# teshnizi/GraphEnvs

Measured on AMD Instinct MI355X. Metric: env-steps/sec (whole node), ShortestPath-v0 n=64 m=192 batch=65536, 1/2/4/8 GPU, higher is better.
Workload: dtype u64; 1 GPU; ShortestPath-v0 n_nodes=64 n_edges=192 weighted, 65536 env slots per GPU, random valid actions on device, same-step autoreset (seed-exact G(n,m)+features on device); envs_per_gpu=65536, prefetch_period=0, episodes_finished_per_gpu=6165512, settle_steps=128, parallelism=batch shard x1, no collective

## Files before the change

graphenvs_amd/csrc/ge_features.h:

```cpp
#pragma once
#include "ge_params.h"
#include "ge_platform.h"
#include "ge_reset.h"

struct GeFctx {
  uint64_t *abits; int *rowptr; uint16_t *scw;
  uint64_t *quads; uint32_t *rq; int zq;
  uint8_t *c8;
  double *sigma, *delta, *coeff, *bcw;
  double *bcw0; int wave_f64;
  double *bc, *clos;
  double *prx, *prn, *sinv, *diff, *diff2, *clus;
  uint8_t *mark;
  uint16_t *ord, *lvl;
};

GE_DEV GeFctx ge_carve_f(const GeParams &P, int tid) {
  unsigned char *s = ge_dyn_smem();
  const GeLdsF &L = P.ldsf;
  const int n = P.n, an = ((n * 8 + 15) & ~15) / 8;
  GeFctx c;
  c.rowptr = (int *)(s + L.rowptr); c.quads = (uint64_t *)(s + L.colw); c.c8 = (uint8_t *)(s + L.colw); c.rq = (uint32_t *)(s + L.rq); c.zq = L.zq;
  c.bc = (double *)(s + L.bc); c.clos = (double *)(s + L.clos);
  unsigned char *w = s + L.wave0 + (tid >> 6) * L.wave_stride;
  const int bcw_at = P.W <= GE_BCW_REG_W ? n : 3 * n + 1;
  c.sigma = (double *)(w + L.w_sigma); c.delta = c.sigma + n; c.coeff = c.sigma + 2 * n; c.bcw = c.sigma + bcw_at;
  c.mark = (uint8_t *)(w + L.w_mark); c.ord = (uint16_t *)(w + L.w_ord); c.lvl = (uint16_t *)(w + L.w_lvl);
  c.bcw0 = (double *)(s + L.wave0 + L.w_sigma) + bcw_at; c.wave_f64 = L.wave_stride / 8;
  c.abits = (uint64_t *)(s + L.abits); c.scw = (uint16_t *)(s + L.scw);
  c.prx = (double *)(s + L.prx); c.prn = c.prx + an; c.sinv = c.prx + 2 * an; c.diff = c.prx + 3 * an; c.diff2 = c.prx + 4 * an; c.clus = (double *)(s + L.clus);
  return c;
}

#ifndef GE_PR_CH
#define GE_PR_CH 4
#endif
#ifndef GE_FABL
#define GE_FABL 0
#endif
#if defined(GE_STAMPS) && !defined(GE_EMU)
#define GE_FSTAMP_DECL unsigned long long fs_acc[8] = {0, 0, 0, 0, 0, 0, 0, 0}, fs_t = clock64(), fs_src = 0, fs_lev = 0; int fs_k = 7
#define GE_FSTAMP(k) do { const unsigned long long now_ = clock64(); fs_acc[fs_k] += now_ - fs_t; fs_t = now_; fs_k = (k); if ((k) == 6) fs_src++; if ((k) == 1) fs_lev++; } while (0)
#define GE_FSTAMP_OUT do { if (env == 0 && part == 0 && tid == 0) { for (int k_ = 0; k_ < 8; k_++) ge_stamp_buf[16 + k_] = fs_acc[k_]; ge_stamp_buf[24] = fs_src; ge_stamp_buf[25] = fs_lev; } } while (0)
#else
#define GE_FSTAMP_DECL do { } while (0)
#define GE_FSTAMP(k) do { } while (0)
#define GE_FSTAMP_OUT do { } while (0)
#endif
GE_HOSTDEV int ge_feat_workgroups(int feat_parts) { return feat_parts > 1 ? feat_parts + 1 : 1; }
#ifndef GE_BW_TWO_ABOVE
#define GE_BW_TWO_ABOVE 256
#endif
#ifndef GE_BW_U
#define GE_BW_U 1
#endif
template <bool BWD, int U>
GE_DEV void ge_brandes_walk_u(const GeFctx &c, int k0, int k1, int lane, bool store) {
  for (int kb = k0; kb < k1; kb += U * GE_WAVE) {
    bool on[U]; int v[U]; uint32_t q0[U], nq[U]; double sv[U], acc[U]; uint64_t q[U];
#pragma unroll
    for (int u = 0; u < U; u++) { const int k = kb + u * GE_WAVE + lane; on[u] = k < k1; v[u] = (int)c.ord[on[u] ? k : k0]; }
#pragma unroll
    for (int u = 0; u < U; u++) { const uint32_t r = c.rq[v[u]]; q0[u] = r & 0xffffu; nq[u] = on[u] ? (r >> 16) : 0u; sv[u] = BWD ? c.sigma[v[u]] : 1.0; acc[u] = 0.0; }
#pragma unroll
    for (int u = 0; u < U; u++) q[u] = c.quads[nq[u] ? q0[u] : (uint32_t)c.zq];
    for (uint32_t i = 0; ge_ballot(i < nq[0] || (U > 1 && i < nq[U - 1])) != 0ull;) {
      i++;
      uint64_t qn[U];
#pragma unroll
      for (int u = 0; u < U; u++) qn[u] = c.quads[i < nq[u] ? q0[u] + i : (uint32_t)c.zq];
#pragma unroll
      for (int u = 0; u < U; u++) {
        const uint32_t lo = (uint32_t)q[u], hi = (uint32_t)(q[u] >> 32);
        const int w0 = (int)(lo & 0xffffu), w1 = (int)(lo >> 16), w2 = (int)(hi & 0xffffu), w3 = (int)(hi >> 16);
        const double f0 = c.coeff[w0], f1 = c.coeff[w1], f2 = c.coeff[w2], f3 = c.coeff[w3];
        if (!BWD) { c.mark[w0] = 1; c.mark[w1] = 1; c.mark[w2] = 1; c.mark[w3] = 1; }
        if (BWD) { acc[u] += sv[u] * f0; acc[u] += sv[u] * f1; acc[u] += sv[u] * f2; acc[u] += sv[u] * f3; }
        else { acc[u] += f0; acc[u] += f1; acc[u] += f2; acc[u] += f3; }
        q[u] = qn[u];
      }
    }
#pragma unroll
    for (int u = 0; u < U; u++) if (on[u] && store) (BWD ? c.delta : c.sigma)[v[u]] = acc[u];
  }
}
template <bool BWD>
GE_DEV void ge_brandes_walk(const GeFctx &c, int k0, int k1, int lane, bool store, bool two) {
  if (GE_BW_U > 1 && two && k1 - k0 > GE_WAVE) ge_brandes_walk_u<BWD, GE_BW_U>(c, k0, k1, lane, store); else ge_brandes_walk_u<BWD, 1>(c, k0, k1, lane, store);
}

GE_DEV void ge_features_generic_env(const GeParams &P, int env, int part, int nparts) {
  const int tid = ge_tid_fresh(), nthreads = ge_bdim();
  const int lane = tid & (GE_WAVE - 1), wv = tid >> 6, nwaves = P.ldsf.waves;
  const bool search_wave = wv < nwaves;
  const int n = P.n, W = P.W, E = P.E, F = P.F, t = P.env_type;
  const ge_buffers &G = P.buf;
  const int64_t nbase = (int64_t)env * n, ebase = (int64_t)env * E;
  GeFctx c = ge_carve_f(P, tid);
  const bool node_part = nparts > 1 && part == nparts;
  const bool node_role = node_part || nparts == 1, brandes_role = !node_part;
  if (node_role) { const uint64_t *arows = G.adj_bits + nbase * W; for (int i = tid; i < n * W; i += nthreads) c.abits[i] = arows[i]; }
  const bool closed = P.complete && P.ng == n;
  const bool trivial = closed || node_part;
  uint8_t *c8 = c.c8;
  const int32_t *grow = G.row_ptr + (int64_t)env * (n + 1);
  const uint16_t *gcolw = G.colw + ebase;
  for (int v = tid; v <= n; v += nthreads) c.rowptr[v] = grow[v];
  if (closed) { for (int idx = tid; idx < E; idx += nthreads) c8[idx] = G.scode[ebase + idx]; }
  else if (brandes_role) {
    uint16_t *q16 = (uint16_t *)c.quads;
    for (int v = tid; v < n; v += nthreads) {
      const int r0 = grow[v], r1 = grow[v + 1], q0 = (r0 + 3 * v) >> 2, nq = (r1 - r0 + 3) >> 2;
      c.rq[v] = (uint32_t)q0 | ((uint32_t)nq << 16);
      for (int i = 0; i < nq; i++) {
        uint32_t e[4];
#pragma unroll
        for (int j = 0; j < 4; j++) { const int k = r0 + 4 * i + j; const uint32_t x = gcolw[k < r1 ? k : r0]; e[j] = k < r1 ? (x >> 4) : (uint32_t)n; }
        c.quads[q0 + i] = (uint64_t)(e[0] | (e[1] << 16)) | ((uint64_t)(e[2] | (e[3] << 16)) << 32);
      }
    }
    if (tid < 4) q16[4 * c.zq + tid] = (uint16_t)n;
  }
  ge_sync();
  if (node_role && !closed) for (int v = tid; v < n; v += nthreads)
    for (int k = c.rowptr[v]; k < c.rowptr[v + 1]; k++) {
      const uint16_t e = gcolw[k];
      c.scw[c.rowptr[v] + ge_rank_below(c.abits + v * W, e >> 4)] = e;
    }
  const bool bcw_reg = W <= GE_BCW_REG_W;
  double bcr[GE_BCW_REG_W];
#pragma unroll
  for (int j = 0; j < GE_BCW_REG_W; j++) bcr[j] = 0.0;
  if (brandes_role && !bcw_reg && search_wave) for (int v = lane; v < n; v += GE_WAVE) c.bcw[v] = 0.0;
  ge_sync();
  if (trivial && !node_part) for (int v = tid; v < n; v += nthreads) c.clos[v] = (((double)n - 1.0) / (double)(n - 1)) * (((double)n - 1.0) / (double)(n - 1));
  const bool two = n > GE_BW_TWO_ABOVE;
  GE_FSTAMP_DECL;
  for (int s = part * nwaves + wv; s < n && !trivial && search_wave; s += nwaves * nparts) {
    GE_FSTAMP(6);
    for (int v = lane; v < n; v += GE_WAVE) { c.sigma[v] = (v == s) ? 1.0 : 0.0; c.delta[v] = 0.0; c.coeff[v] = (v == s) ? 1.0 : 0.0; c.mark[v] = 0; }
    const uint32_t rs = c.rq[s];
    const int deg_s = c.rowptr[s + 1] - c.rowptr[s];
    { const uint16_t *row = (const uint16_t *)(c.quads + (rs & 0xffffu)); for (int i = lane; i < deg_s; i += GE_WAVE) c.ord[1 + i] = row[i]; }
    if (lane == 0) { c.coeff[n] = 0.0; c.mark[n] = 0; c.ord[0] = (uint16_t)s; c.lvl[0] = 0; c.lvl[1] = 1; c.lvl[2] = (uint16_t)(1 + deg_s); }
    ge_wave_sync();
    int d = deg_s ? 1 : 0, reach = 1 + deg_s, lp = 0, lo = deg_s ? 1 : 0, hi = 1 + deg_s; int64_t tot = deg_s;
    const uint32_t *sig_hi = (const uint32_t *)c.sigma + 1;
    for (;;) {
      GE_FSTAMP(1);
      if (!(GE_FABL & 1) && d > 0) ge_brandes_walk<false>(c, lo, hi, lane, true, two);
      ge_wave_sync();
      GE_FSTAMP(0);
      int found = 0;
      for (int w0 = 0; w0 < n; w0 += 4 * GE_WAVE) {
        uint32_t m[4], sh[4];
#pragma unroll
        for (int j = 0; j < 4; j++) { const int w = w0 + GE_WAVE * j + lane; const bool in = w < n; m[j] = c.mark[in ? w : n]; sh[j] = sig_hi[2 * (in ? w : 0)]; }
#pragma unroll
        for (int j = 0; j < 4; j++) if (w0 + GE_WAVE * j < n) {
          const int w = w0 + GE_WAVE * j + lane; const bool in = w < n;
          const bool isnew = in && m[j] != 0u && sh[j] == 0u;
          const uint64_t b = ge_ballot(isnew);
          if (isnew) c.ord[hi + found + ge_mbcnt(b)] = (uint16_t)w;
          if (in) c.mark[w] = 0;
          found += ge_popc64(b);
        }
      }
      if (!found) break;
      for (int k = lp + lane; k < lo; k += GE_WAVE) c.coeff[c.ord[k]] = 0.0;
      for (int k = lo + lane; k < hi; k += GE_WAVE) { const int v = c.ord[k]; c.coeff[v] = c.sigma[v]; }
      d++; lp = lo; lo = hi; hi += found; reach += found; tot += (int64_t)d * found;
      if (lane == 0) c.lvl[d + 1] = (uint16_t)hi;
      ge_wave_sync();
    }
    for (int k = lp + lane; k < lo; k += GE_WAVE) c.coeff[c.ord[k]] = 0.0;
    ge_wave_sync();
    for (int lev = d; lev >= 2; lev--) {
      GE_FSTAMP(3);
      const int l0 = c.lvl[lev], l1 = c.lvl[lev + 1], l2 = lev < d ? (int)c.lvl[lev + 2] : l1, p0 = c.lvl[lev - 1];
      for (int k = l1 + lane; k < l2; k += GE_WAVE) c.coeff[c.ord[k]] = 0.0;
      for (int k = l0 + lane; k < l1 && !(GE_FABL & 2); k += GE_WAVE) { const int v = c.ord[k]; c.coeff[v] = (1.0 + c.delta[v]) / c.sigma[v]; if (!bcw_reg) c.bcw[v] += c.delta[v]; }
      ge_wave_sync();
      GE_FSTAMP(4);
      if (!(GE_FABL & 4)) ge_brandes_walk<true>(c, p0, l0, lane, true, two);
      ge_wave_sync();
    }
    GE_FSTAMP(5);
    if (!bcw_reg) { const int l1 = c.lvl[2]; for (int k = 1 + lane; k < l1; k += GE_WAVE) { const int v = c.ord[k]; c.bcw[v] += c.delta[v]; } }
    if (bcw_reg) {
#pragma unroll
      for (int j = 0; j < GE_BCW_REG_W; j++) { const int v = lane + GE_WAVE * j; if (j < W) bcr[j] += (v < n && v != s) ? c.delta[v] : 0.0; }
    }
    if (lane == 0) {
      double cc = 0.0;
      if (tot > 0 && n > 1) { cc = ((double)reach - 1.0) / (double)tot; double sc = ((double)reach - 1.0) / (double)(n - 1); cc *= sc; }
      c.clos[s] = cc;
    }
    ge_wave_sync();
  }
  GE_FSTAMP(7);
  GE_FSTAMP_OUT;
  if (bcw_reg && brandes_role && search_wave) {
#pragma unroll
    for (int j = 0; j < GE_BCW_REG_W; j++) { const int v = lane + GE_WAVE * j; if (j < W && v < n) c.bcw[v] = bcr[j]; }
  }
  ge_sync();
  if (brandes_role) for (int v = tid; v < n; v += nthreads) { double acc = 0.0; for (int w = 0; w < nwaves; w++) acc += c.bcw0[w * c.wave_f64 + v]; c.bc[v] = acc; }
  ge_sync();
  if (nparts > 1) {
    if (!node_part) {
      for (int v = tid; v < n; v += nthreads) G.feat_scratch[((int64_t)env * nparts + part) * n + v] = c.bc[v];
      for (int v = tid; v < n; v += nthreads) if ((v % (nwaves * nparts)) / nwaves == part) G.x[(nbase + v) * F + P.nflag + 2] = (float)c.clos[v];
      ge_sync();
      return;
    }
  }
  if (n > 2 && nparts == 1) { double scale = 1.0 / (double)((int64_t)(n - 1) * (int64_t)(n - 2)); for (int v = tid; v < n; v += nthreads) c.bc[v] *= scale; }
  double *clus = c.clus;
  for (int i = tid; i < n; i += nthreads) {
    int64_t common = 0, dg = c.rowptr[i + 1] - c.rowptr[i];
    for (int k = c.rowptr[i]; k < c.rowptr[i + 1]; k++) {
      int j;
      if (closed) { const int q = k - c.rowptr[i]; j = q < i ? q : q + 1; } else j = c.scw[k] >> 4;
      for (int w = 0; w < W; w++) common += ge_popc64(c.abits[i * W + w] & c.abits[j * W + w]);
    }
    int64_t t8 = 8 * common, dt = 2 * dg, db = dg;
    clus[i] = (t8 == 0) ? 0.0 : (double)t8 / (double)((dt * (dt - 1) - 2 * db) * 2);
  }
  const bool prw = (t == GE_TSP);
  const double pinit = 1.0 / (double)n;
  int ndang = 0;
  for (int k0 = 0; k0 < n; k0 += GE_WAVE) {
    int i = k0 + lane;
    ndang += ge_popc64(ge_ballot(i < n && c.rowptr[i + 1] == c.rowptr[i]));
  }
  double *wl = (double *)(ge_dyn_smem() + P.ldsf.wl);
  if (tid < 16) wl[tid] = ge_wlut(tid);
  ge_sync();
  for (int i = tid; i < n; i += nthreads) {
    double S = 0.0;
    for (int k = c.rowptr[i]; k < c.rowptr[i + 1]; k++) S += (prw ? (P.spatial ? G.sw64[ebase + k] : wl[closed ? (int)c8[k] : (int)(c.scw[k] & 15)]) : 1.0) * 1.0;
    c.sinv[i] = (S != 0.0) ? 1.0 / S : 0.0;
    c.prx[i] = pinit;
  }
  ge_sync();
  const double alpha = 0.85, oma = 1 - alpha, tol = 1.0e-6;
  double *xc = c.prx, *xw = c.prn, *dc = c.diff, *dw = c.diff2;
  bool conv = false;
  for (int it = 0; it < ((GE_FABL & 8) ? 1 : 100) && !conv; it++) {
    double dsum = 0.0;
    if (ndang) { bool first = true; for (int i = 0; i < n; i++) if (c.rowptr[i + 1] == c.rowptr[i]) { dsum = first ? xc[i] : dsum + xc[i]; first = false; } }
    for (int i = tid; i < n; i += nthreads) {
      double acc = 0.0;
      const int r0 = c.rowptr[i], r1 = c.rowptr[i + 1];
      for (int k0 = r0; k0 < r1; k0 += GE_PR_CH) {
        int jn[GE_PR_CH], cd[GE_PR_CH]; double sv[GE_PR_CH], xv[GE_PR_CH], wv[GE_PR_CH];
#pragma unroll
        for (int q = 0; q < GE_PR_CH; q++) {
          const int kk = k0 + q < r1 ? k0 + q : r0;
          if (closed) { const int qq = kk - r0; jn[q] = qq < i ? qq : qq + 1; cd[q] = (int)c8[kk]; }
          else { const uint32_t e = (uint32_t)c.scw[kk]; jn[q] = (int)(e >> 4); cd[q] = (int)(e & 15u); }
        }
#pragma unroll
        for (int q = 0; q < GE_PR_CH; q++) {
          sv[q] = c.sinv[jn[q]]; xv[q] = xc[jn[q]];
          wv[q] = prw ? (P.spatial ? G.sw64[ebase + (k0 + q < r1 ? k0 + q : r0)] : wl[cd[q]]) : 1.0;
        }
#pragma unroll
        for (int q = 0; q < GE_PR_CH; q++) if (k0 + q < r1) acc += (sv[q] * wv[q]) * xv[q];
      }
      double xn = alpha * (acc + dsum * pinit) + oma * pinit;
      xw[i] = xn;
      dc[i] = __builtin_fabs(xn - xc[i]);
    }
    ge_sync();
    const double err = ge_pw<5>(dc, n, lane);
    { double *t_ = xc; xc = xw; xw = t_; t_ = dc; dc = dw; dw = t_; }
    if (err < (double)n * tol) conv = true;
  }

  for (int v = tid; v < n; v += nthreads) {
    float *xr = G.x + (nbase + v) * F + P.nflag;
    xr[0] = (float)(2.0 * (double)(c.rowptr[v + 1] - c.rowptr[v]));
    if (nparts == 1) { xr[1] = (float)c.bc[v]; xr[2] = (float)c.clos[v]; }
    xr[3] = (float)xc[v]; xr[4] = (float)clus[v];
  }
  ge_sync();
}

#ifndef GE_F64_LV
#define GE_F64_LV 12
#endif
#ifndef GE_F64_INV
#define GE_F64_INV 128
#endif
#ifndef GE_F64_ABL
#define GE_F64_ABL 0
#endif
#ifndef GE_F64_U
#define GE_F64_U 2
#endif
#ifndef GE_F64_L2POP
#define GE_F64_L2POP 1
#endif
#define GE_F64_THREADS 256
#define GE_F64_WAVES 4
#define GE_F64_SB 8
#define GE_F64_LST 16
#define GE_F64_ITEMS 16
static_assert(GE_F64_LV + 1 <= GE_F64_LST, "level starts");
static_assert(GE_F64_INV <= 256, "path counts are kept as bytes");
#define GE_F64_SS 65
#define GE_F64_SG 68
#define GE_F64_A_S 0
#define GE_F64_A_SIG (GE_F64_A_S + GE_F64_SB * GE_F64_SS * 8)
#define GE_F64_A_LVL (GE_F64_A_SIG + GE_F64_SB * GE_F64_SG)
#define GE_F64_A_ORD (GE_F64_A_LVL + GE_F64_LV * GE_F64_SB * 8)
#define GE_F64_A_LST (GE_F64_A_ORD + GE_F64_SB * 64)
#define GE_F64_A_BYTES (GE_F64_A_LST + GE_F64_SB * GE_F64_LST)
#define GE_F64_W_INV 512
#define GE_F64_W_CLOS (GE_F64_W_INV + GE_F64_INV * 8)
#define GE_F64_W_AREA (GE_F64_W_CLOS + 512)
#define GE_F64_W_BYTES (GE_F64_W_AREA + GE_F64_WAVES * GE_F64_A_BYTES)

GE_HOSTDEV int ge_f64_node_wave_bytes(int E, int tsp) { return 512 + 4 * 512 + (tsp ? ((E + 15) & ~15) : 0); }
GE_HOSTDEV int ge_f64_pre_off(int E, int tsp, int nblk) {
  int o = GE_F64_W_BYTES;
  const int nd = GE_F64_WAVES * ge_f64_node_wave_bytes(E, tsp), pf = (nblk + 2) * 4;
  if (nd > o) o = nd;
  if (pf > o) o = pf;
  return (o + 15) & ~15;
}
GE_HOSTDEV int ge_f64_bytes(int E, int tsp, int nblk) { return ge_f64_pre_off(E, tsp, nblk) + GE_F64_ITEMS * 4 * 4 + 16; }

template <int BASE>
GE_DEV void ge_f64_next_bits(uint32_t &b, int (&idx)[GE_F64_U]) {
#pragma unroll
  for (int j = 0; j < GE_F64_U; j++) {
#ifdef GE_EMU
    idx[j] = b ? BASE + __builtin_ctz(b) : 64;
#else
    uint32_t z;
    asm("v_ffbl_b32 %0, %1" : "=v"(z) : "v"(b));
    idx[j] = (int)((z < (uint32_t)(64 - BASE) ? z : (uint32_t)(64 - BASE)) + (uint32_t)BASE);
#endif
    b &= b - 1u;
  }
}
GE_DEV uint32_t ge_f64_sum_counts(const uint8_t *row, uint64_t p) {
  uint32_t acc = 0u;
  for (uint32_t b = (uint32_t)p; b;) {
    int ix[GE_F64_U]; uint32_t r[GE_F64_U];
    ge_f64_next_bits<0>(b, ix);
#pragma unroll
    for (int j = 0; j < GE_F64_U; j++) r[j] = row[ix[j]];
#pragma unroll
    for (int j = 0; j < GE_F64_U; j++) acc += r[j];
  }
  for (uint32_t b = (uint32_t)(p >> 32); b;) {
    int ix[GE_F64_U]; uint32_t r[GE_F64_U];
    ge_f64_next_bits<32>(b, ix);
#pragma unroll
    for (int j = 0; j < GE_F64_U; j++) r[j] = row[ix[j]];
#pragma unroll
    for (int j = 0; j < GE_F64_U; j++) acc += r[j];
  }
  return acc;
}
#ifndef GE_F64_COEFF
#define GE_F64_COEFF 0
#endif
template <int BASE>
GE_DEV double ge_f64_sum_coeff_half(const uint8_t *sigrow, const double *Srow, const double *inv, uint32_t b, double acc) {
#if GE_F64_COEFF
  while (b) {
    int ix[GE_F64_U]; double sw[GE_F64_U];
    ge_f64_next_bits<BASE>(b, ix);
#pragma unroll
    for (int j = 0; j < GE_F64_U; j++) sw[j] = Srow[ix[j]];
#pragma unroll
    for (int j = 0; j < GE_F64_U; j++) acc += sw[j];
  }
  return acc;
#endif
  while (b) {
    int ix[GE_F64_U]; uint32_t sg[GE_F64_U]; double sw[GE_F64_U], iv[GE_F64_U];
    ge_f64_next_bits<BASE>(b, ix);
#pragma unroll
    for (int j = 0; j < GE_F64_U; j++) { sg[j] = sigrow[ix[j]]; sw[j] = Srow[ix[j]]; }
#pragma unroll
    for (int j = 0; j < GE_F64_U; j++) iv[j] = inv[sg[j]];
#pragma unroll
    for (int j = 0; j < GE_F64_U; j++) acc += iv[j] + sw[j];
  }
  return acc;
}

GE_DEV void ge_f64_walk_env(const GeParams &P, int env, int *ovf_flag, int32_t *work_count, int32_t *work_list, int env_global) {
  const int tid = ge_tid_fresh();
  const int lane = tid & (GE_WAVE - 1), wv = tid >> 6;
  const int n = P.n, F = P.F;
  const ge_buffers &G = P.buf;
  const int64_t nbase = (int64_t)env * n;
  unsigned char *const sm = ge_dyn_smem();
  uint64_t *const abits = (uint64_t *)sm;
  double *const inv = (double *)(sm + GE_F64_W_INV), *const clos = (double *)(sm + GE_F64_W_CLOS);
  unsigned char *const area = sm + GE_F64_W_AREA + wv * GE_F64_A_BYTES;
  double *const S = (double *)(area + GE_F64_A_S);
  uint8_t *const sig = (uint8_t *)(area + GE_F64_A_SIG);
  uint64_t *const lvl = (uint64_t *)(area + GE_F64_A_LVL);
  uint8_t *const ord = (uint8_t *)(area + GE_F64_A_ORD), *const lst = (uint8_t *)(area + GE_F64_A_LST);
  GE_STAMP(11);
  if (wv == 0) abits[lane] = lane < n ? G.adj_bits[nbase + lane] : 0ull;
  if (tid == 0) *ovf_flag = 0;
  for (int i = tid; i < GE_F64_INV; i += GE_F64_THREADS) inv[i] = i > 0 ? 1.0 / (double)i : 0.0;
  ge_sync();
  GE_STAMP(12);
  const int sl = lane >> 3, o = lane & 7;
  const uint64_t below_o = (1ull << (8 * o)) - 1ull;
  uint8_t *const sigrow = sig + sl * GE_F64_SG; double *const Srow = S + sl * GE_F64_SS;
  uint8_t *const ordrow = ord + sl * 64, *const lstrow = lst + sl * GE_F64_LST;
  double bc = 0.0;
  bool ovf = false;
  for (int r = 0; r < 2; r++) {
    const int s = 32 * r + GE_F64_SB * wv + sl;
    const bool src = s < n;
    uint64_t vis = src ? (1ull << s) : 0ull, cur = vis;
    int D = 0, reach = 1, start = src ? 1 : 0, Dw = 0; int64_t tot = 0;
    if (o == 0) { lvl[sl] = cur; lstrow[0] = 0; lstrow[1] = (uint8_t)start; if (src) ordrow[0] = (uint8_t)s; }
    uint32_t rlo[8], rhi[8];
#pragma unroll
    for (int j = 0; j < 8; j++) { const uint64_t rw = abits[8 * o + j]; rlo[j] = (uint32_t)rw; rhi[j] = (uint32_t)(rw >> 32); }
    for (int d = 1; !(GE_F64_ABL & 32); d++) {
      const uint32_t cb = (uint32_t)(cur >> (8 * o)) & 0xffu;
      uint32_t nlo = 0u, nhi = 0u;
#pragma unroll
      for (int j = 0; j < 8; j++) { const uint32_t m = 0u - ((cb >> j) & 1u); nlo |= m & rlo[j]; nhi |= m & rhi[j]; }
      nlo = ge_oct_or32(nlo); nhi = ge_oct_or32(nhi);
      const uint64_t nw = (((uint64_t)nhi << 32) | (uint64_t)nlo) & ~vis;
      if (!ge_ballot(nw != 0ull)) break;
      Dw = d;
      vis |= nw; cur = nw;
      if (nw) {
        const int cnt = ge_popc64(nw);
        D = d; reach += cnt; tot += (int64_t)d * cnt;
        if (d < GE_F64_LV) {
          if (o == 0) lvl[d * GE_F64_SB + sl] = nw;
          int pos = start + ge_popc64(nw & below_o);
          for (uint32_t nb = (uint32_t)(nw >> (8 * o)) & 0xffu; nb; nb &= nb - 1u) ordrow[pos++] = (uint8_t)(8 * o + __builtin_ctz(nb));
        } else ovf = true;
        start += cnt;
      }
      if (o == 0 && d + 1 < GE_F64_LST) lstrow[d + 1] = (uint8_t)start;
    }
    if (o == 0 && src) {
      double cl = 0.0;
      if (tot > 0 && n > 1) { cl = ((double)reach - 1.0) / (double)tot; cl *= ((double)reach - 1.0) / (double)(n - 1); }
      clos[s] = cl;
    }
    if (r > 0) ge_sync();
    for (int i = lane; i < GE_F64_SB * GE_F64_SG / 4; i += GE_WAVE) ((uint32_t *)sig)[i] = 0u;
    for (int i = lane; i < GE_F64_SB * GE_F64_SS; i += GE_WAVE) S[i] = 0.0;
    ge_wave_sync();
    if (o == 0 && src) sigrow[s] = 1;
    { const int lo = lstrow[1], hi = Dw >= 1 ? (int)lstrow[2] : lo; for (int k = lo + o; k < hi; k += 8) sigrow[ordrow[k]] = 1; }
    const bool deep = ge_ballot(ovf) != 0ull;
#if GE_F64_L2POP
    if (Dw >= 2 && !deep && !(GE_F64_ABL & 1)) {
      const uint64_t l1 = lvl[GE_F64_SB + sl];
      for (int k = lstrow[2] + o, hi = lstrow[3]; k < hi; k += 8) {
        const int v = ordrow[k]; const uint32_t acc = (uint32_t)ge_popc64(abits[v] & l1);
        sigrow[v] = (uint8_t)acc;
        if (GE_F64_INV < 64 && acc >= (uint32_t)GE_F64_INV) ovf = true;
      }
    }
#endif
    ge_wave_sync();
    for (int d = GE_F64_L2POP ? 3 : 2; d <= Dw && !deep && !(GE_F64_ABL & 1); d++) {
      const int lo = lstrow[d], hi = lstrow[d + 1];
      const uint64_t prev = lvl[(d - 1) * GE_F64_SB + sl];
      for (int k = lo + o; ge_ballot(k < hi) != 0ull; k += 8) {
        if (k < hi) {
          const int v = ordrow[k];
          const uint64_t p = abits[v] & prev;
          const uint32_t acc = ge_f64_sum_counts(sigrow, p);
          sigrow[v] = (uint8_t)(acc < 255u ? acc : 255u);
          if (acc >= (uint32_t)GE_F64_INV) ovf = true;
        }
      }
      ge_wave_sync();
    }
    const bool deep2 = ge_ballot(ovf) != 0ull;
#if GE_F64_COEFF
    if (!deep2) for (int i = lane; i < GE_F64_SB * 64; i += GE_WAVE) { const int a = (i >> 6) * GE_F64_SS + (i & 63), g = (i >> 6) * GE_F64_SG + (i & 63); S[a] = inv[sig[g] < GE_F64_INV ? sig[g] : 0]; }
    ge_wave_sync();
#endif
    for (int d = Dw - 1; d >= 1 && !deep2 && !(GE_F64_ABL & 2); d--) {
      const bool mine = d < D;
      const int lo = lstrow[d], hi = mine ? lstrow[d + 1] : lo;
      const uint64_t next = lvl[(d + 1) * GE_F64_SB + sl];
      for (int k = lo + o; ge_ballot(k < hi) != 0ull; k += 8) {
        if (k < hi) {
          const int v = ordrow[k];
          const uint64_t sc = abits[v] & next;
          double acc = ge_f64_sum_coeff_half<0>(sigrow, Srow, inv, (uint32_t)sc, 0.0);
          acc = ge_f64_sum_coeff_half<32>(sigrow, Srow, inv, (uint32_t)(sc >> 32), acc);
#if GE_F64_COEFF
          acc += inv[sigrow[v]];
#endif
          Srow[v] = acc;
        }
      }
      ge_wave_sync();
    }
    if (ovf) *ovf_flag = 1;
    ge_sync();
    if (wv == 0 && !(GE_F64_ABL & 16)) {
#pragma unroll 1
      for (int w = 0; w < GE_F64_WAVES; w++) {
        const unsigned char *const aw = sm + GE_F64_W_AREA + w * GE_F64_A_BYTES;
        const uint8_t *const sgw = (const uint8_t *)(aw + GE_F64_A_SIG) + lane; const double *const Sw = (const double *)(aw + GE_F64_A_S) + lane;
        uint32_t sg[GE_F64_SB]; double sv[GE_F64_SB];
#pragma unroll
        for (int k = 0; k < GE_F64_SB; k++) { sg[k] = sgw[GE_F64_SG * k]; sv[k] = Sw[GE_F64_SS * k]; }
#if GE_F64_COEFF
#pragma unroll
        for (int k = 0; k < GE_F64_SB; k++) sv[k] -= inv[sg[k] < GE_F64_INV ? sg[k] : 0u];
#endif
#pragma unroll
        for (int k = 0; k < GE_F64_SB; k++) bc += (32 * r + GE_F64_SB * w + k != lane) ? (double)sg[k] * sv[k] : 0.0;
      }
    }
  }
  GE_STAMP(14);
  if (*ovf_flag) {
    if (tid == 0) { int k = atomicAdd(&work_count[0], 1); work_list[k] = env_global; }
    ge_sync();
    return;
  }
  if (wv == 0 && lane < n) {
    if (n > 2) bc *= 1.0 / (double)((int64_t)(n - 1) * (int64_t)(n - 2));
    float *xr = G.x + (nbase + lane) * F + P.nflag;
    xr[1] = (float)bc; xr[2] = (float)clos[lane];
  }
  ge_sync();
  GE_STAMP(17);
}

GE_DEV void ge_f64_node_env(const GeParams &P, int env, unsigned char *area, int lane) {
  const int n = P.n, E = P.E, F = P.F, t = P.env_type;
  const ge_buffers &G = P.buf;
  const int64_t nbase = (int64_t)env * n, ebase = (int64_t)env * E;
  const bool prw = (t == GE_TSP);
  uint64_t *const abits = (uint64_t *)area;
  double *const cx = (double *)(area + 512), *const cy = cx + 64, *const csinv = cx + 128, *const cdiff = cx + 192;
  uint8_t *const scode = area + 512 + 4 * 512;
  const bool live = lane < n;
  const uint64_t adj = live ? G.adj_bits[nbase + lane] : 0ull;
  const int deg = ge_popc64(adj);
  abits[lane] = adj;
  if (prw) for (int i = lane; i < E; i += GE_WAVE) scode[i] = G.scode[ebase + i];
  ge_wave_sync();
  double clus = 0.0, x = 0.0;
  if (live && !(GE_F64_ABL & 8)) {
    int64_t common = 0;
    for (uint64_t r = adj; r; r &= r - 1) common += ge_popc64(adj & abits[ge_ctz64(r)]);
    const int64_t t8 = 8 * common, dt = 2 * (int64_t)deg, db = deg;
    clus = (t8 == 0) ? 0.0 : (double)t8 / (double)((dt * (dt - 1) - 2 * db) * 2);
  }
  int rp = 0;
  if (prw) { int incl = ge_wave_incl_scan(deg, lane); rp = incl - deg; }
  double S = 0.0;
  { int k = 0; for (uint64_t r = adj; r; r &= r - 1, k++) S += (prw ? ge_wlut(scode[rp + k]) : 1.0) * 1.0; }
  const double sinv = (S != 0.0) ? 1.0 / S : 0.0;
  const double pinit = 1.0 / (double)n;
  const double alpha = 0.85, oma = 1 - alpha, tol = 1.0e-6;
  const uint64_t dangling = ge_ballot(live && deg == 0);
  x = pinit;
  csinv[lane] = sinv;
  uint32_t nb4[4] = {0u, 0u, 0u, 0u}; uint64_t rest = adj;
  { int k = 0; for (; rest && k < 16; rest &= rest - 1, k++) nb4[k >> 2] |= (uint32_t)ge_ctz64(rest) << (8 * (k & 3)); }
  bool conv = false;
  for (int it = 0; it < ((GE_F64_ABL & 4) ? 1 : 100) && !conv; it++) {
    cx[lane] = x; cy[lane] = sinv * x;
    ge_wave_sync();
    double dsum = 0.0;
    { bool first = true; for (uint64_t r = dangling; r; r &= r - 1) { double xv = cx[ge_ctz64(r)]; dsum = first ? xv : dsum + xv; first = false; } }
    double xn = 0.0;
    if (live) {
      double acc = 0.0;
      if (prw) { int k = 0; for (uint64_t r = adj; r; r &= r - 1, k++) { const int j = ge_ctz64(r); acc += (csinv[j] * ge_wlut(scode[rp + k])) * cx[j]; } }
      else {
#pragma unroll
        for (int k = 0; k < 16; k++) { const double yv = cy[(nb4[k >> 2] >> (8 * (k & 3))) & 63u]; acc += (k < deg) ? yv : 0.0; }
        for (uint64_t r = rest; r; r &= r - 1) acc += cy[ge_ctz64(r)];
      }
      xn = alpha * (acc + dsum * pinit) + oma * pinit;
    }
    cdiff[lane] = live ? __builtin_fabs(xn - x) : 0.0;
    ge_wave_sync();
    const double err = ge_pw<0>(cdiff, n, lane);
    x = xn;
    ge_wave_sync();
    if (err < (double)n * tol) conv = true;
  }
  if (live) {
    float *xr = G.x + (nbase + lane) * F + P.nflag;
    xr[0] = (float)(2.0 * (double)deg); xr[3] = (float)x; xr[4] = (float)clus;
  }
  ge_wave_sync();
}


GE_DEV int ge_slot_class(const GeRagged &R, int env) { return (int)ge_uniform_u32((uint32_t)R.slot_class[env]); }

#ifndef GE_GEN_WPS
#define GE_GEN_WPS 0
#endif
#if GE_GEN_WPS > 0
#define GE_GEN_KERNEL GE_KERNEL_LB(512, GE_GEN_WPS)
#else
#define GE_GEN_KERNEL GE_KERNEL
#endif
template <bool RAGGED>
GE_GEN_KERNEL ge_k_features(GeParams P, GeRagged R, GeRun run, int pre_off, int bucket) {
  int *pre = (int *)(ge_dyn_smem() + pre_off);
  const bool queue = run.items == GE_ITEMS_QUEUE, list = run.items == GE_ITEMS_LIST;
  if (list) ge_wave_priority(GE_PRIO_PROBE);
  int count = list ? P.buf.work_count[0] : P.B;
  if (list && count > 0) ge_wave_priority(0);
  if (queue) {
    if (ge_tid() < GE_WAVE) ge_queue_prefix_wave(P, pre, ge_tid());
    ge_sync();
    count = pre[(P.B + GE_STEP_BLOCK - 1) / GE_STEP_BLOCK];
  }
  const int fparts = (list && !RAGGED) ? 1 : P.feat_parts;
  const int nparts = ge_feat_workgroups(fparts);
  for (int q = ge_bid(); q < count * nparts; q += ge_gdim()) {
    const int item = q / nparts, part = q % nparts;
    const int env = queue ? ge_queue_slot(P, pre, item) : (list ? P.buf.work_list[item] : item);
    if constexpr (RAGGED) {
      const int cls = ge_slot_class(R, env);
      const GeParams &C = R.classes[cls];
      if (bucket >= 0 && C.bucket != bucket) continue;
      if (queue && part == 0 && ge_tid() == 0) ge_finish_item(P, run, env);
      if (part < ge_feat_workgroups(C.feat_parts)) ge_features_generic_env(C, env - R.class_start[cls], part, C.feat_parts);
    } else {
      if (queue && part == 0 && ge_tid() == 0) ge_finish_item(P, run, env);
      ge_features_generic_env(P, env, part, fparts);
    }
  }
}

template <bool RAGGED>
GE_KERNEL ge_k_feat_combine(GeParams P, GeRagged R, GeRun run) {
  int *pre = (int *)ge_dyn_smem();
  const bool queue = run.items == GE_ITEMS_QUEUE, list = run.items == GE_ITEMS_LIST;
  int count = list ? P.buf.work_count[0] : P.B;
  if (queue) {
    if (ge_tid() < GE_WAVE) ge_queue_prefix_wave(P, pre, ge_tid());
    ge_sync();
    count = pre[(P.B + GE_STEP_BLOCK - 1) / GE_STEP_BLOCK];
  }
  const int nmax = P.n;
  for (int64_t g = (int64_t)ge_bid() * ge_bdim() + ge_tid(); g < (int64_t)count * nmax; g += (int64_t)ge_gdim() * ge_bdim()) {
    const int item = (int)(g / nmax), v = (int)(g % nmax);
    int env = queue ? ge_queue_slot(P, pre, item) : (list ? P.buf.work_list[item] : item);
    int cls = 0;
    if constexpr (RAGGED) { cls = R.slot_class[env]; env -= R.class_start[cls]; }
    const GeParams &C = RAGGED ? R.classes[cls] : P;
    const int n = C.n, nparts = C.feat_parts;
    if (v >= n || nparts == 1) continue;
    double acc = 0.0;
    for (int p = 0; p < nparts; p++) acc += C.buf.feat_scratch[((int64_t)env * nparts + p) * n + v];
    if (n > 2) acc *= 1.0 / (double)((int64_t)(n - 1) * (int64_t)(n - 2));
    C.buf.x[((int64_t)env * n + v) * C.F + C.nflag + 1] = (float)acc;
  }
}

#ifndef GE_F64_WPS
#define GE_F64_WPS 6
#endif
#if GE_F64_WPS > 0
#define GE_F64_KERNEL GE_KERNEL_LB(GE_F64_THREADS, GE_F64_WPS)
#else
#define GE_F64_KERNEL GE_KERNEL
#endif
template <bool RAGGED>
GE_F64_KERNEL ge_k_features64(GeParams P, GeRagged R, GeRun run, int tail_off) {
  const int nblk = (P.B + GE_STEP_BLOCK - 1) / GE_STEP_BLOCK;
  int *const pre = (int *)ge_dyn_smem();
  int *const items = (int *)(ge_dyn_smem() + tail_off);
  int *const ovf_flag = items + GE_F64_ITEMS * 4;
  const bool queue = run.items == GE_ITEMS_QUEUE;
  const int nseed2 = (GE_SEED_SPLIT && queue) ? run.seed_split : 0;
  if (nseed2 > 0 && ge_bid() < nseed2) {
    ge_wave_priority(GE_PRIO_SEED2);
    for (int g0 = ge_bid() * GE_SEED2_ITEMS;; g0 += nseed2 * GE_SEED2_ITEMS) {
      const int tid = ge_tid_fresh();
      if (tid < GE_WAVE) ge_queue_prefix_wave(P, pre, tid);
      ge_sync();
      const int count = pre[nblk];
      if (g0 >= count) break;
      const int q = g0 + tid;
      uint32_t sb = 0xffffffffu;
      if (tid < GE_SEED2_ITEMS && q < count) {
        const int env = ge_queue_slot(P, pre, q);
        sb = (uint32_t)env * GE_SEED_DEPTH + (uint32_t)((P.buf.episode[env] + run.seed_ahead) % GE_SEED_DEPTH);
        ge_advance_episode(P, env);
      }
      ge_sync();
      if (tid < GE_SEED2_ITEMS) ge_seed_pass2_group(P, ge_dyn_smem(), sb, tid);
      ge_sync();
    }
    return;
  }
  const int bid = ge_bid() - nseed2, gdim = ge_gdim() - nseed2;
  int count = P.B;
  for (int base = 0;; base += GE_F64_ITEMS) {
    const int tid = ge_tid_fresh();
    if (queue) {
      if (tid < GE_WAVE) ge_queue_prefix_wave(P, pre, tid);
      ge_sync();
      count = pre[nblk];
    }
    const int total = count + (count + 3) / 4;
    if (bid + (int64_t)base * gdim >= total) break;
    if (tid < GE_F64_ITEMS * 4) {
      const int64_t q = bid + (int64_t)(base + (tid >> 2)) * gdim;
      const int sub = tid & 3;
      int qi = -1;
      if (q < count) qi = sub == 0 ? (int)q : -1;
      else if (q < total) { const int64_t k = 4 * (q - count) + sub; qi = k < count ? (int)k : -1; }
      items[tid] = qi < 0 ? -1 : (queue ? ge_queue_slot(P, pre, qi) : qi);
    }
    ge_sync();
    for (int i = 0; i < GE_F64_ITEMS; i++) {
      const int64_t q = bid + (int64_t)(base + i) * gdim;
      if (q >= total) break;
      if (q < count) {
        const int env = items[4 * i];
        if (queue && nseed2 == 0 && ge_tid() == 0) ge_finish_item(P, run, env);
        if constexpr (RAGGED) {
          const int cls = ge_slot_class(R, env);
          const GeParams &C = R.classes[cls];
          if (C.n > 64) {
            if (ge_tid() == 0) { int k = atomicAdd(&P.buf.work_count[0], 1); P.buf.work_list[k] = env; }
            continue;
          }
          ge_f64_walk_env(C, env - R.class_start[cls], ovf_flag, P.buf.work_count, P.buf.work_list, env);
        } else {
          ge_f64_walk_env(P, env, ovf_flag, P.buf.work_count, P.buf.work_list, env);
        }
      } else {
        const int t2 = ge_tid_fresh();
        const int wv = t2 >> 6, lane = t2 & (GE_WAVE - 1);
        const int env = items[4 * i + wv];
        if (env >= 0) {
          if constexpr (RAGGED) {
            const int cls = ge_slot_class(R, env);
            const GeParams &C = R.classes[cls];
            if (C.n <= 64) ge_f64_node_env(C, env - R.class_start[cls], ge_dyn_smem() + wv * ge_f64_node_wave_bytes(R.f64_tsp_e, C.env_type == GE_TSP), lane);
          } else {
            ge_f64_node_env(P, env, ge_dyn_smem() + wv * ge_f64_node_wave_bytes(P.E, P.env_type == GE_TSP), lane);
          }
        }
        ge_sync();
      }
    }
    ge_sync();
  }
}
```

Before: 424.5 million env-steps/s.

## Group BFS sources by reachable-set size to balance wave work in betweenness walk

Before the betweenness-centrality BFS walk, each source node gets a key from the size of its two-hop reachable set. Sources are ranked by that key within each half of 64, and the ranking permutes which wave and sub-lane handles which source, so the 8 sources sharing a wave have similar BFS depth and work. This is meant to cut the divergence and idle time where a wave waits on its slowest source. The cost is a per-env ranking pass (a 32-way compare per lane), extra LDS for the map, and a gather through readlane-decoded addresses in the accumulation step.

```diff
diff --git a/graphenvs_amd/csrc/ge_features.h b/graphenvs_amd/csrc/ge_features.h
--- a/graphenvs_amd/csrc/ge_features.h
+++ b/graphenvs_amd/csrc/ge_features.h
@@ -303,6 +303,9 @@
 #ifndef GE_F64_L2POP
 #define GE_F64_L2POP 1
 #endif
+#ifndef GE_F64_SRCGROUP
+#define GE_F64_SRCGROUP 1
+#endif
 #define GE_F64_THREADS 256
 #define GE_F64_WAVES 4
 #define GE_F64_SB 8
@@ -320,7 +323,8 @@
 #define GE_F64_A_BYTES (GE_F64_A_LST + GE_F64_SB * GE_F64_LST)
 #define GE_F64_W_INV 512
 #define GE_F64_W_CLOS (GE_F64_W_INV + GE_F64_INV * 8)
-#define GE_F64_W_AREA (GE_F64_W_CLOS + 512)
+#define GE_F64_W_SRC (GE_F64_W_CLOS + 512)
+#define GE_F64_W_AREA (GE_F64_W_SRC + (GE_F64_SRCGROUP ? 64 : 0))
 #define GE_F64_W_BYTES (GE_F64_W_AREA + GE_F64_WAVES * GE_F64_A_BYTES)
 
 GE_HOSTDEV int ge_f64_node_wave_bytes(int E, int tsp) { return 512 + 4 * 512 + (tsp ? ((E + 15) & ~15) : 0); }
@@ -395,6 +399,41 @@
   }
   return acc;
 }
+
+GE_HOSTDEV uint32_t ge_f64_src_key(const uint64_t *rows, int n, int s) {
+  uint32_t key = 64u;
+  if (s < n) {
+    uint64_t r = rows[s];
+    for (uint64_t b = r; b; b &= b - 1ull) r |= rows[__builtin_ctzll(b)];
+    key = (uint32_t)__builtin_popcountll(r & ~(1ull << s));
+  }
+  return (key << 6) | (uint32_t)s;
+}
+GE_HOSTDEV int ge_f64_src_rank(const uint32_t *keys, int s) {
+  const uint32_t *const half = keys + (s & 32); const uint32_t mine = keys[s];
+  int rank = 0;
+  for (int j = 0; j < 32; j++) rank += half[j] < mine ? 1 : 0;
+  return rank;
+}
+GE_DEV int ge_f64_source_map(const uint64_t *rows, int n, int lane, uint32_t *keys, uint8_t *srcmap) {
+  keys[lane] = ge_f64_src_key(rows, n, lane);
+  ge_wave_sync();
+  const int rank = ge_f64_src_rank(keys, lane);
+  srcmap[(lane & 32) + rank] = (uint8_t)lane;
+  return rank;
+}
+#ifdef GE_EMU
+GE_KERNEL ge_k_emu_source_map(const uint64_t *rows, int n, uint8_t *out) {
+  const int lane = ge_tid();
+  uint64_t *const abits = (uint64_t *)ge_dyn_smem(); uint32_t *const keys = (uint32_t *)(abits + 64); uint8_t *const maps = (uint8_t *)(keys + 64);
+  abits[lane] = lane < n ? rows[lane] : 0ull;
+  ge_wave_sync();
+  const int rank = ge_f64_source_map(abits, n, lane, keys, maps);
+  ge_wave_sync();
+  out[lane] = maps[lane]; out[64 + lane] = (uint8_t)rank;
+}
+extern "C" void ge_emu_f64_source_map(const uint64_t *rows, int n, uint8_t *out) { GE_LAUNCH(ge_k_emu_source_map, 1, 64, 512 + 256 + 64, nullptr, rows, n, out); }
+#endif
 
 GE_DEV void ge_f64_walk_env(const GeParams &P, int env, int *ovf_flag, int32_t *work_count, int32_t *work_list, int env_global) {
   const int tid = ge_tid_fresh();
@@ -412,6 +451,14 @@
   uint8_t *const ord = (uint8_t *)(area + GE_F64_A_ORD), *const lst = (uint8_t *)(area + GE_F64_A_LST);
   GE_STAMP(11);
   if (wv == 0) abits[lane] = lane < n ? G.adj_bits[nbase + lane] : 0ull;
+#if GE_F64_SRCGROUP
+  uint8_t *const srcmap = sm + GE_F64_W_SRC;
+  int srcpos = 0;
+  if (wv == 0) {
+    ge_wave_sync();
+    srcpos = ge_f64_source_map(abits, n, lane, (uint32_t *)area, srcmap);
+  }
+#endif
   if (tid == 0) *ovf_flag = 0;
   for (int i = tid; i < GE_F64_INV; i += GE_F64_THREADS) inv[i] = i > 0 ? 1.0 / (double)i : 0.0;
   ge_sync();
@@ -423,7 +470,11 @@
   double bc = 0.0;
   bool ovf = false;
   for (int r = 0; r < 2; r++) {
+#if GE_F64_SRCGROUP
+    const int s = srcmap[32 * r + GE_F64_SB * (GE_F64_WAVES - 1 - wv) + sl];
+#else
     const int s = 32 * r + GE_F64_SB * wv + sl;
+#endif
     const bool src = s < n;
     uint64_t vis = src ? (1ull << s) : 0ull, cur = vis;
     int D = 0, reach = 1, start = src ? 1 : 0, Dw = 0; int64_t tot = 0;
@@ -515,6 +566,28 @@
     }
     if (ovf) *ovf_flag = 1;
     ge_sync();
+#if GE_F64_SRCGROUP
+    if (wv == 0 && !(GE_F64_ABL & 16)) {
+      const int p = srcpos, base = GE_F64_W_AREA + (GE_F64_WAVES - 1 - (p >> 3)) * GE_F64_A_BYTES;
+      const uint32_t at = (uint32_t)(base + GE_F64_A_SIG + (p & 7) * GE_F64_SG) | ((uint32_t)(base + GE_F64_A_S + (p & 7) * GE_F64_SS * 8) << 16);
+      static_assert(GE_F64_W_BYTES < 65536, "two LDS offsets in one word");
+#pragma unroll 1
+      for (int i0 = 0; i0 < 32; i0 += GE_F64_SB) {
+        uint32_t sg[GE_F64_SB]; double sv[GE_F64_SB];
+#pragma unroll
+        for (int k = 0; k < GE_F64_SB; k++) {
+          const uint32_t a = ge_readlane_u32(at, 32 * r + i0 + k);
+          sg[k] = ((const uint8_t *)(sm + (a & 0xffffu)))[lane]; sv[k] = ((const double *)(sm + (a >> 16)))[lane];
+        }
+#if GE_F64_COEFF
+#pragma unroll
+        for (int k = 0; k < GE_F64_SB; k++) sv[k] -= inv[sg[k] < GE_F64_INV ? sg[k] : 0u];
+#endif
+#pragma unroll
+        for (int k = 0; k < GE_F64_SB; k++) bc += (32 * r + i0 + k != lane) ? (double)sg[k] * sv[k] : 0.0;
+      }
+    }
+#else
     if (wv == 0 && !(GE_F64_ABL & 16)) {
 #pragma unroll 1
       for (int w = 0; w < GE_F64_WAVES; w++) {
@@ -531,6 +604,7 @@
         for (int k = 0; k < GE_F64_SB; k++) bc += (32 * r + GE_F64_SB * w + k != lane) ? (double)sg[k] * sv[k] : 0.0;
       }
     }
+#endif
   }
   GE_STAMP(14);
   if (*ovf_flag) {
```

Result: no change. 428.4 million env-steps/s (median of 6 runs) (+0.9%).
